# pingpongshow/RIA

Measured on AMD Instinct MI355X. Metric: frames/s demod+LDPC-decoded, OFDM QAM16 R1/2 1024-FFT, higher is better.
Workload: dtype f32; 1 GPU; OFDM QAM16 R1/2 + LDPC min-sum, Watterson moderate fading 20 dB, 4400000 frames (100000 per step per GPU), full decodeFixedFrame; frame_samples=18432, batch_per_gpu=100000, channel=2

## Files before the change

ria_amd/csrc/ldpc_fast.hip.h:

```cpp
#pragma once
#include <hip/hip_runtime.h>
#include <stdint.h>

#include <type_traits>

#include "../../include/ria_gpu.h"
#include "devmath.h"
#include "ldpc_kernels.hip.h"

namespace ria {

struct ShapeR12 {
    static constexpr int NR = 6, NC = 6;
    static constexpr int kCascadeWaves = 3;
    static constexpr int kCv = 24;
    static constexpr bool kStateExit = true;
    static constexpr int ne(int r) { constexpr int t[NR] = {6, 6, 5, 4, 2, 1}; return t[r]; }
    static constexpr int nm(int r) { constexpr int t[NR] = {6, 5, 4, 2, 1, 1}; return t[r]; }
    static constexpr int dv(int r) { constexpr int t[NC] = {5, 4, 4, 4, 4, 4}; return t[r]; }
};
struct ShapeR13 {
    static constexpr int NR = 6, NC = 6;
    static constexpr int kCascadeWaves = 3;
    static constexpr int kCv = 24;
// ... 43 lines not shown

template <class S>
struct ShapeInfo {
    static constexpr int row_off(int r) { int t = 0; for (int i = 0; i < r; ++i) t += S::ne(i); return t; }
    static constexpr int col_off(int r) { int t = 0; for (int i = 0; i < r; ++i) t += S::dv(i); return t; }
    static constexpr int mix_off(int r) { int t = 0; for (int i = 0; i < r; ++i) t += S::ne(i) - S::nm(i); return t; }
    static constexpr int TS = row_off(S::NR);
    static constexpr int TD = col_off(S::NC);
    static constexpr int TM = mix_off(S::NR);
    static constexpr int tot_word = 64 * TS;
    static constexpr int zero_word = tot_word + 64 * S::NC;
    static constexpr int dump_word = zero_word + 64;
    static constexpr int big_word = dump_word + 64;
    static constexpr int words = big_word + 64;
    static constexpr int lds_bytes = ((words < 1296 ? 1296 : words) * 4 + 15) & ~15;
    static constexpr int copy_words = 2 * S::NR + (S::NR + 1) / 2;
    static constexpr int exit_lds_bytes = lds_bytes + (S::kStateExit ? 256 * copy_words : 0);
};

template <int B, int E, class F>
__device__ __forceinline__ void static_for(F&& f) {
    if constexpr (B < E) {
        f(std::integral_constant<int, B>{});
        static_for<B + 1, E>(f);
    }
}

struct FastCode {
    int k, m, max_iter, bytes_per_cw;
    const uint16_t* row_addr;
    const uint16_t* col_addr;
    const uint16_t* check_at;
// ... 104 lines not shown
            if constexpr (N >= 5) { mid = med3_abs(w[4], lo, mid); lo = min_abs(w[4], lo); }
        }
    }
}
__device__ __forceinline__ uint32_t bfi(uint32_t mask, uint32_t a, uint32_t b) { return (mask & a) | (~mask & b); }

__device__ __forceinline__ float llr_canon(float x) {
    x = (x < 1e30f) ? x : 1e30f;
    x = (-1e30f < x) ? x : -1e30f;
    return x + 0.0f;
}

#ifndef RIA_SINGLE_PREFETCH
#define RIA_SINGLE_PREFETCH 2
#endif
constexpr int kExitFirst = 22, kExitStride = 24;
template <class S, int NCV = (kCvRegs ? 1024 : S::kCv), int PF = RIA_SINGLE_PREFETCH, bool EX = false>
__device__ inline int fast_decode(FastState<S>& st, const FastCode& c, unsigned char* __restrict__ lds,
                                  float factor, int max_iter, int lane, bool* ok, unsigned int* exits = nullptr) {
    using I = ShapeInfo<S>;
    static_assert(!EX || S::kStateExit, "the shape has no room for the state copy");
    const uint32_t lane4 = lds_addr(lds) + static_cast<uint32_t>(lane) * 4u;
    const uint32_t kAbs = 0x7fffffffu;
    const uint32_t m0base = lds_addr(lds);
    static_for<0, S::NR>([&](auto R_) __attribute__((always_inline)) {
        constexpr int r = decltype(R_)::value;
#pragma unroll
        for (int s = 0; s < S::ne(r); ++s) {
            const float v0 = 0.0f;
            if (I::row_off(r) + s < NCV) st.cv[I::row_off(r) + s] = v0;
            else lds_sf(lane4 + 256u * (I::row_off(r) + s), v0);
        }
    });
#pragma unroll
    for (int r = 0; r < S::NC; ++r) lds_sf(lane4 + 4u * (I::tot_word + 64 * r), st.li[r]);
    lds_sf(lane4 + 4u * I::zero_word, 0.0f);
    lds_sf(lane4 + 4u * I::big_word, kPadTotal);
#pragma unroll
    for (int r = 0; r < S::NR; ++r) { st.pv[r] = st.lp[r]; st.pt[r] = 0.0f; }
    wave_sync();
    float hi = __builtin_inff();
    int it = 0;
    bool success = false;
    auto iteration = [&](auto SNAP_) __attribute__((always_inline)) -> int {
        constexpr bool SNAP = decltype(SNAP_)::value;
        uint32_t syn = 0;
        uint32_t sb = 0, sd = 0;
        float tt[I::TS];
        auto gather_round = [&](auto G_) __attribute__((always_inline)) {
            constexpr int g = decltype(G_)::value;
            if constexpr (g < S::NR) {
#pragma unroll
                for (int s = 0; s < S::ne(g); ++s) tt[I::row_off(g) + s] = lds_f(st.rv[I::row_off(g) + s]);
            }
        };
        static_for<0, PF>([&](auto G_) __attribute__((always_inline)) { gather_round(G_); });
        static_for<0, S::NR>([&](auto R_) __attribute__((always_inline)) {
            constexpr int r = decltype(R_)::value;
            constexpr int NE = S::ne(r);
            constexpr int off = I::row_off(r);
            gather_round(std::integral_constant<int, r + PF>{});
            float t[NE], cold[NE];
// ... 27 lines not shown
            syn |= par;
            const uint32_t dS = bfi(kAbs, f2u(min1) ^ f2u(min2), sgn);
            float o[NE];
#pragma unroll
            for (int s = 0; s < NE; ++s) o[s] = u2f(dS ^ f2u(__builtin_amdgcn_fmed3f(v[s], min2, -min2))) * factor;
            lds_store_tid_n<NE, 256 * off, 256>(m0base, o);
            static_for<0, NE>([&](auto S_) __attribute__((always_inline)) {
                constexpr int s = decltype(S_)::value;
                if constexpr (off + s < NCV) st.cv[off + s] = o[s];
            });
            {
                const float c2v = u2f(dS ^ f2u(__builtin_amdgcn_fmed3f(pvr, min2, -min2))) * factor;
                const float tot = st.lp[r] + c2v;
                st.pv[r] = tot - c2v;
                st.pt[r] = tot;
                if constexpr (SNAP) {
                    static_assert(NE + 1 <= 8, "16 bits per round");
                    const uint32_t ma = f2u(min1 * factor) & kAbs, mb = f2u(min2 * factor) & kAbs;
                    uint32_t bits = (f2u(c2v) >> 31) | (((f2u(c2v) & kAbs) != ma) ? 2u : 0u);
#pragma unroll
                    for (int s = 0; s < NE; ++s) bits = (bits << 2) | (f2u(o[s]) >> 31) | (((f2u(o[s]) & kAbs) != ma) ? 2u : 0u);
                    const uint32_t ca = lane4 + static_cast<uint32_t>(I::lds_bytes) + 256u * (2 * r);
                    sd |= (f2u(lds_f(ca)) ^ ma) | (f2u(lds_f(ca + 256u)) ^ mb);
                    lds_sf(ca, u2f(ma));
                    lds_sf(ca + 256u, u2f(mb));
                    sb = (r & 1) ? (sb | (bits << 16)) : bits;
                    if constexpr ((r & 1) || r == S::NR - 1) {
                        const uint32_t cb = lane4 + static_cast<uint32_t>(I::lds_bytes) + 256u * (2 * S::NR + r / 2);
                        sd |= f2u(lds_f(cb)) ^ sb;
                        lds_sf(cb, u2f(sb));
                    }
                }
            }
        });
        if (it > 0 && __ballot(static_cast<int>(syn) < 0) == 0ull) return 1;
        if constexpr (SNAP) {
            if (it != kExitFirst && __ballot(sd != 0u) == 0ull) return 2;
        }
        hi = 50.0f;
        wave_sync();
        constexpr int NCE = []() constexpr { int n = 0; for (int r = 0; r < S::NC; ++r) if (S::dv(r) > 0) n = r + 1; return n; }();
        float totv[NCE > 0 ? NCE : 1];
        static_for<0, NCE>([&](auto R_) __attribute__((always_inline)) {
            constexpr int r = decltype(R_)::value;
            constexpr int DV = S::dv(r);
            constexpr int off = I::col_off(r);
            float cv[DV > 0 ? DV : 1];
#pragma unroll
            for (int d = 0; d < DV; ++d) cv[d] = lds_f(st.cs[off + d]);
            float tot = st.li[r];
#pragma unroll
            for (int d = 0; d < DV; ++d) tot = tot + cv[d];
            totv[r] = tot;
        });
        static_for<0, (NCE + 5) / 6>([&](auto G_) __attribute__((always_inline)) {
            constexpr int g0 = 6 * decltype(G_)::value, gn = (NCE - g0 < 6) ? NCE - g0 : 6;
            float tv[gn];
#pragma unroll
            for (int i = 0; i < gn; ++i) tv[i] = totv[g0 + i];
            lds_store_tid_n<gn, 4 * (I::tot_word + 64 * g0), 256>(m0base, tv);
        });
        wave_sync();
        return 0;
    };
    int snap_at = (EX && exits != nullptr) ? kExitFirst : 0x7fffffff;
    int status = 0;
    for (;;) {
        const int stop = snap_at < max_iter ? snap_at : max_iter;
        for (; it < stop; ++it) {
            status = iteration(std::false_type{});
            if (status != 0) break;
        }
        if (status != 0 || it >= max_iter) break;
        if constexpr (!EX) break;
        else {
            status = iteration(std::true_type{});
            if (status != 0) break;
            ++it;
            snap_at += kExitStride;
        }
    }
    if (status == 1) { success = true; --it; }
    if constexpr (EX) {
        if (status == 2) {
            if (lane == 0) atomicAdd(exits, 1u);
            *ok = false;
            return max_iter;
        }
    }
    if (!success) {
        uint32_t syn = 0;
        static_for<0, S::NR>([&](auto R_) __attribute__((always_inline)) {
            constexpr int r = decltype(R_)::value;
            constexpr int off = I::row_off(r);
            uint32_t par = f2u(st.pt[r]);
// ... 60 lines not shown
    uint8_t* info_out;
    ria_decode_status* status;
    const uint16_t* crc_bit;
    const uint16_t* crc_init;
    DecodeCtl* ctl;
    unsigned int* entries;
    unsigned int* best;
    unsigned int* list1;
    CwResult* res;
    uint8_t* res_bytes;
    CascadeWin* win;
    float* staged;
    unsigned int* l1idx;
    unsigned int* l1hash;
    uint32_t* seed_ws;
    int state_exit;
    __device__ unsigned int* exit_counter(int which) const { return state_exit ? &ctl->exits[which] : nullptr; }
};

constexpr int kStageFloats = 12 * 64;
constexpr int kStageFrameFloats = 2688;

constexpr float kIdleRowLlr = 1e30f;

template <class S>
__device__ inline void fast_gather_llr(FastState<S>& st, const FastCode& c, const float* fl, const uint16_t* gather,
                                       int cw, int lane) {
    lane = opaque_lane(lane);
#pragma unroll
    for (int r = 0; r < S::NC; ++r) {
        const uint32_t j = c.col_at[lane + 64 * r];
        st.li[r] = (j != 0xFFFFu) ? llr_canon(fl[gather[cw * 648 + j]]) : 0.0f;
// ... 12 lines not shown
#pragma unroll
    for (int r = 0; r < S::NC; ++r) st.li[r] = src[r * 64 + lane];
#pragma unroll
    for (int r = 0; r < S::NR; ++r) st.lp[r] = src[(S::NC + r) * 64 + lane];
}

__device__ inline void fast_publish(CwResult* res, unsigned fc, int f, bool ok, int it, int lane) {
    if (lane == 0) {
        res[fc].iters[f] = static_cast<uint16_t>(it);
        __hip_atomic_store(&res[fc].state[f], static_cast<uint8_t>(ok ? 2 : 1), __ATOMIC_RELAXED, __HIP_MEMORY_SCOPE_AGENT);
    }
}

template <class S, int NCV = S::kCv, bool EX = false>
__device__ inline void fast_unit(FastState<S>& st, const FastDecodeArgs& A, unsigned char* lds, unsigned fc, int f, int lane,
                                 const float* staged = nullptr, unsigned int* exits = nullptr) {
    const FastCode& c = A.c;
    if (staged) fast_load_staged(st, staged, lane);
    else fast_gather_llr(st, c, A.llr + static_cast<size_t>(fc >> 2) * A.llr_stride, A.gather, fc & 3, lane);
    bool ok;
    int it = fast_decode<S, NCV, RIA_SINGLE_PREFETCH, EX>(st, c, lds, kFactors[f], c.max_iter, lane, &ok, exits);
    if (ok) fast_pack(st, c, lds, A.res_bytes + (static_cast<size_t>(fc) * kNumFactors + f) * c.bytes_per_cw,
                      c.bytes_per_cw, lane);
    fast_publish(A.res, fc, f, ok, it, lane);
}

#ifndef RIA_PRIMARY_NCV
#define RIA_PRIMARY_NCV 0
#endif
template <class S>
__global__ __launch_bounds__(64) void fast_primary_kernel(FastDecodeArgs A) {
    extern __shared__ __attribute__((aligned(16))) unsigned char smem[];
    const int lane = threadIdx.x;
    const unsigned b = blockIdx.x, g = b >> 5, r = b & 31u, cw = r >> 3, x = r & 7u;
    const unsigned frame = 8u * g + x;
    if (frame >= static_cast<unsigned>(A.n_frames)) return;
// ... 55 lines not shown
                const uint32_t k = c.check_at[lane + 64 * (r - S::NC)];
                v = (k != 0xFFFFu) ? llr_canon(fr[A.gather[cw * 648 + c.k + k]]) : kIdleRowLlr;
            }
            dst[r * 64 + lane] = v;
        }
        if (wave == 0) {
            const uint32_t h = fast_hash16(fr, A.gather, cw, lane);
            if (lane == 0) A.l1hash[i] = h;
        }
    }
}

#ifndef RIA_EAGER_FACTORS
#define RIA_EAGER_FACTORS 0
#endif
template <class S, bool EX = false>
__global__ __launch_bounds__(64) void fast_phase0_kernel(FastDecodeArgs A) {
    extern __shared__ __attribute__((aligned(16))) unsigned char smem[];
    const int lane = threadIdx.x;
    const unsigned n_list1 = A.ctl->n_list1, total = n_list1 * 4u;
    if (blockIdx.x >= total) return;
    FastState<S> st;
    fast_load_tables(st, A.c, smem, lane);
    unsigned guard = 0;
    for (;;) {
        RIA_QUEUE_GUARD(guard, total, A.ctl)
        unsigned u = atomicAdd(&A.ctl->next_z, lane == 0 ? 1u : 0u);
        u = __builtin_amdgcn_readfirstlane(u);
        if (u >= total) break;
#if RIA_EAGER_FACTORS
        const unsigned entry = u >> 2;
        const int t = 1 + static_cast<int>(u & 3u);
        const unsigned fc = A.list1[entry];
#else
        const unsigned tq = u / n_list1, entry = u - tq * n_list1;
        const int t = 1 + static_cast<int>(tq);
        const unsigned fc = A.list1[entry];
        bool done = false;
        for (int k = 1; k < t; ++k) {
            const unsigned sk = __hip_atomic_load(&A.res[fc].state[k], __ATOMIC_RELAXED, __HIP_MEMORY_SCOPE_AGENT);
            done = done || __builtin_amdgcn_readfirstlane(sk) == 2u;
        }
        if (done) continue;
#endif
        fast_unit<S, S::kCv, EX>(st, A, smem, fc, t, lane, A.staged + static_cast<size_t>(entry) * kStageFloats,
                                 A.exit_counter(kExitsPhase0));
    }
}

__global__ void fast_chain_kernel(FastDecodeArgs A) {
    int frame = blockIdx.x * blockDim.x + threadIdx.x;
    if (frame >= A.n_frames) return;
    const int bpc = A.c.bytes_per_cw;
    int f = 0;
    ria_decode_status* s = A.status + frame;
    for (int cw = 0; cw < 4; ++cw) {
        const unsigned fc = static_cast<unsigned>(frame) * 4u + cw;
        const CwResult r = A.res[fc];
        int accept = -1, attempts = 1, iters = r.iters[f];
        if (r.state[f] == 2) accept = f;
        else {
// ... 52 lines not shown
    for (int r = 0; r < S::NC; ++r) {
        const uint32_t q = c.col_at[lane + 64 * r];
        const float nz = (noise && q != 0xFFFFu) ? normal[q] : 0.0f;
        st.li[r] = (q != 0xFFFFu) ? llr_canon(tf(base_i[r], nz)) : 0.0f;
    }
#pragma unroll
    for (int r = 0; r < S::NR; ++r) {
        const uint32_t i = c.check_at[lane + 64 * r];
        const float nz = (noise && i != 0xFFFFu) ? normal[c.k + i] : 0.0f;
        st.lp[r] = (i != 0xFFFFu) ? llr_canon(tf(base_p[r], nz)) : kIdleRowLlr;
    }
    wave_sync();
    return factor;
}

template <class S, bool EX = false>
__global__ __launch_bounds__(64) __attribute__((amdgpu_waves_per_eu(S::kCascadeWaves))) void fast_cascade_kernel(FastDecodeArgs A) {
    extern __shared__ __attribute__((aligned(16))) unsigned char smem[];
    const FastCode& c = A.c;
    const int lane = threadIdx.x;
    float* msg = reinterpret_cast<float*>(smem);
    const unsigned int n_entries = A.ctl->n_entries;
    const unsigned int total = n_entries * kCascadeGroups;
    if (total == 0) return;
    FastState<S> st;
    fast_load_tables(st, c, smem, lane);
    unsigned guard = 0;
    for (;;) {
        RIA_QUEUE_GUARD(guard, total, A.ctl)
        unsigned int u = atomicAdd(&A.ctl->next_unit, lane == 0 ? 1u : 0u);
        u = __builtin_amdgcn_readfirstlane(u);
// ... 10 lines not shown
            const unsigned int a = a0 + static_cast<unsigned>(j);
            if (a >= kRetryAttempts) break;
            if (j > 0) {
                b = __hip_atomic_load(&A.best[e], __ATOMIC_RELAXED, __HIP_MEMORY_SCOPE_AGENT);
                b = __builtin_amdgcn_readfirstlane(b);
                if (b < a) break;
            }
            fast_load_staged(st, A.staged + static_cast<size_t>(li) * kStageFloats, lane);
            float bi[S::NC], bp[S::NR];
#pragma unroll
            for (int r = 0; r < S::NC; ++r) bi[r] = st.li[r];
#pragma unroll
            for (int r = 0; r < S::NR; ++r) bp[r] = st.lp[r];
            float factor = fast_perturb(st, c, bi, bp, reinterpret_cast<uint32_t*>(msg), msg + 640, ws, j, static_cast<int>(a), lane);
            bool ok;
            const int it = fast_decode<S, (kCvRegs ? 1024 : S::kCv), RIA_SINGLE_PREFETCH, EX>(st, c, smem, factor, c.max_iter, lane, &ok,
                                                                                     A.exit_counter(kExitsCascade));
            if (!ok) continue;
            unsigned int prev = atomicMin(&A.best[e], lane == 0 ? a : 0xFFFFFFFFu);
            prev = __builtin_amdgcn_readfirstlane(prev);
            if (a < prev) {
                CascadeWin* w = A.win + e;
                bool mine = false;
                for (unsigned spin = 0; spin < (1u << 20); ++spin) {
                    unsigned got = atomicCAS(&w->lock, 0u, lane == 0 ? 1u : 0u);
                    got = __builtin_amdgcn_readfirstlane(got);
                    if (got == 0u) { mine = true; break; }
                    __builtin_amdgcn_s_sleep(1);
                }
                if (!mine) { if (lane == 0) atomicExch(&A.ctl->queue_fault, 1u); break; }
                __threadfence();
                unsigned int cur = __hip_atomic_load(&A.best[e], __ATOMIC_RELAXED, __HIP_MEMORY_SCOPE_AGENT);
// ... 154 lines not shown
```

ria_amd/csrc/recovery_kernels.hip.h:

```cpp
#pragma once
#include <hip/hip_runtime.h>
#include <stdint.h>

#include "fallback_relevance.hpp"
#include "ldpc_fast.hip.h"
#include "sort_exact.hpp"

namespace ria {

struct RecCtx {
    uint8_t* cw;
    uint8_t* fd;
    uint8_t* trial;
    Suspect* sus;
    int* stack;
    uint16_t* sd;
    uint16_t* lists;
    int sus_cap;
    unsigned long long* dbg;
    int bpc;
    const uint16_t* crc_bit;
    const uint16_t* crc_init;
    int lane;
};
// ... 414 lines not shown
    uint8_t* redec_bytes;
};

__global__ void recovery_list_kernel(RecoveryArgs R) {
    int frame = blockIdx.x * blockDim.x + threadIdx.x;
    if (frame >= R.d.n_frames || !R.d.status[frame].needs_recovery) return;
    R.flagged[atomicAdd(R.n_flagged, 1u)] = static_cast<unsigned>(frame);
    if (!R.list_units_now) return;
    for (int cw = 0; cw < 4; ++cw) {
        unsigned fc = static_cast<unsigned>(frame) * 4u + cw, mask = 0;
        for (int f = 1; f <= 4; ++f)
            if (R.d.res[fc].state[f] == 0) mask |= 1u << (f - 1);
        if (mask) R.list2[atomicAdd(R.n_list2, 1u)] = (fc << 4) | mask;
    }
}
template <class S, bool EX = false>
__global__ __launch_bounds__(64) void recovery_fill_kernel(RecoveryArgs R) {
    extern __shared__ __attribute__((aligned(16))) unsigned char smem[];
    const unsigned total = *R.n_list2 * 4u;
    if (blockIdx.x >= total) return;
    FastState<S> st;
    fast_load_tables(st, R.d.c, smem, threadIdx.x);
    unsigned guard = 0;
    for (;;) {
        RIA_QUEUE_GUARD(guard, total, R.d.ctl)
        unsigned u = atomicAdd(R.next_fill, threadIdx.x == 0 ? 1u : 0u);
        u = __builtin_amdgcn_readfirstlane(u);
        if (u >= total) break;
        const unsigned e = R.list2[u >> 2], fc = e >> 4;
        const int f = 1 + static_cast<int>(u & 3u);
        if (!((e >> (f - 1)) & 1u)) continue;
        const FastCode& c = R.d.c;
        const int lane = threadIdx.x;
        unsigned li = kNotListed;
        if (R.d.flags & (RIA_DECODE_PHASE0 | RIA_DECODE_PERTURB)) li = static_cast<unsigned>(__builtin_amdgcn_readfirstlane(static_cast<int>(R.d.l1idx[fc])));
        if (li != kNotListed) fast_load_staged(st, R.d.staged + static_cast<size_t>(li) * kStageFloats, lane);
        else fast_gather_llr(st, c, R.d.llr + static_cast<size_t>(fc >> 2) * R.d.llr_stride, R.d.gather, fc & 3, lane);
        bool ok;
        const int it = fast_decode<S, (kCvRegs ? 1024 : S::kCv), RIA_SINGLE_PREFETCH, EX>(st, c, smem, kFactors[f], c.max_iter, lane, &ok,
                                                                                 R.d.exit_counter(kExitsFill));
        if (ok) fast_pack(st, c, smem, R.d.res_bytes + (static_cast<size_t>(fc) * kNumFactors + f) * c.bytes_per_cw, c.bytes_per_cw, lane);
        fast_publish(R.d.res, fc, f, ok, it, lane);
    }
}
__global__ __launch_bounds__(256) void recovery_gather_kernel(RecoveryArgs R) {
    const unsigned q = blockIdx.x;
    if (q >= *R.n_flagged) return;
    const unsigned frame = R.flagged[q];
    const int bpc = R.d.c.bytes_per_cw, ib = 4 * bpc;
    for (int i = threadIdx.x; i < ib; i += 256) R.info_c[static_cast<size_t>(q) * ib + i] = R.d.info_out[static_cast<size_t>(frame) * ib + i];
    const float* fl = R.d.llr + static_cast<size_t>(frame) * R.d.llr_stride;
    for (int i = threadIdx.x; i < 4 * 648; i += 256) R.rows_c[static_cast<size_t>(q) * 4 * 648 + i] = fl[R.d.gather[i]];
    const int forder[4] = {2, 3, 4, 1};
    if (threadIdx.x < 16) {
        int at = threadIdx.x >> 2, cw = threadIdx.x & 3;
// ... 120 lines not shown
```

ria_amd/csrc/ria_gpu.hip:

```cpp
#include <hip/hip_runtime.h>

#include <cstdarg>
#include <cstdio>
#include <cstdlib>
#include <algorithm>
#include <cstring>
#include <map>
#include <memory>
#include <mutex>
#include <atomic>
#include <chrono>
#include <string>
#include <thread>
#include <vector>

#include "../../include/ria_gpu.h"
#include "host_tables.hpp"
#include "../host/link_adaptation.hpp"
#include "frame_recovery.hpp"
#include "ws_carve.hpp"
#include "device_buffers.hpp"
#include "ldpc_kernels.hip.h"
#include "ldpc_fast.hip.h"
#ifdef RIA_WITH_DUAL_DECODER
// ... 44 lines not shown
    DevBuf d_tx_const;
    DevBuf d_llr_ws;
    FastCode fast{};
    CoreTables ftab;
    DevBuf d_f[5];
    int wave_lds = 0;
    hipStream_t aux_stream[4] = {nullptr, nullptr, nullptr, nullptr};
    hipEvent_t aux_event[5] = {nullptr, nullptr, nullptr, nullptr, nullptr};
    DevBuf d_ctl;
    DevBuf d_seed_ws;
    DevBuf d_decode_ws;
    int ws_frames = 0;
    int split_parts = 0;
    int dual_decoder = 0;
    int fallback_queue_all = 0;
    int state_exit = 0;
    DevBuf d_hstage; PinBuf p_hstage; hipStream_t hstream = nullptr;
    int zc_lds_opted = 0, mc_lds_opted = 0, lts_lds_opted = 0;
    DevBuf d_rec_ws, d_rec_stage; PinBuf p_rec_stage;
    int rec_frames = 0, rec_host_frames = 0;
    Crc16Tables crc;
    DevBuf d_acq_ws; int acq_windows = 0; PinBuf p_acq_ctl;
    DevBuf d_macq_ws; PinBuf p_macq_ctl;
    DevBuf d_burst_ws; PinBuf p_burst_ctl;
    FastCode fast14{}; DevBuf d_f14[5]; int wave_lds14 = 0; bool have14 = false;
    DevBuf d_cw_perm[2];
    DevBuf d_df_ws; PinBuf p_df_ctl;
    std::vector<std::unique_ptr<ria_chase_pool_s>> chase_pools;
    DevBuf d_harq_ws, d_mdf_ws; PinBuf p_mdf_ctl;
};

// ... 66 lines not shown
};
static DecodeWs decode_ws_carve(Carver& c, size_t n_frames, size_t bytes_per_cw) {
    const size_t n4 = 4 * n_frames;
    DecodeWs w;
    w.entries = c.take<unsigned int>(n4);
    w.best = c.take<unsigned int>(n4);
    w.list1 = c.take<unsigned int>(n4);
    w.res = c.take<CwResult>(n4);
    w.res_bytes = c.take<uint8_t>(n4 * kNumFactors * bytes_per_cw);
    w.win = c.take<CascadeWin>(n4);
    w.staged = c.take<float>(n4 * kStageFloats);
    w.l1idx = c.take<unsigned int>(n4);
    w.l1hash = c.take<unsigned int>(n4);
    return w;
}
static hipError_t ensure_decode_ws(ria_gpu_handle h, int n_frames) {
    if (n_frames <= h->ws_frames && h->d_ctl && h->d_seed_ws) return hipSuccess;
    h->ws_frames = 0;
    hipError_t e;
    if (!h->d_ctl) {
        if ((e = h->d_ctl.reserve(kMaxParts * sizeof(DecodeCtl))) != hipSuccess) return e;
        if ((e = hipMemset(h->d_ctl.as<>(), 0, kMaxParts * sizeof(DecodeCtl))) != hipSuccess) { h->d_ctl.release(); return e; }
    }
    if ((e = h->d_seed_ws.reserve(static_cast<size_t>(kMaxParts) * persist_grid_size(false) * kSeedWsWords * sizeof(uint32_t))) != hipSuccess) return e;
    const size_t bpc = h->geo.bytes_per_codeword;
    if ((e = h->d_decode_ws.reserve(carved_size([&](Carver& c) { return decode_ws_carve(c, n_frames, bpc); }))) != hipSuccess) return e;
    h->ws_frames = n_frames;
    return hipSuccess;
}
template <class S, class F>
static void with_state_exit(ria_gpu_handle h, F&& f) {
    if constexpr (S::kStateExit) {
        if (h->state_exit) { f(std::true_type{}, ShapeInfo<S>::exit_lds_bytes); return; }
    }
    f(std::false_type{}, ShapeInfo<S>::lds_bytes);
}
static void set_fast_attributes(int rate, int wb) {
    dispatch_shape(rate, [&](auto s) {
        using S = decltype(s);
        (void)hipFuncSetAttribute(reinterpret_cast<const void*>(fast_primary_kernel<S>), hipFuncAttributeMaxDynamicSharedMemorySize, wb);
        (void)hipFuncSetAttribute(reinterpret_cast<const void*>(fast_phase0_kernel<S>), hipFuncAttributeMaxDynamicSharedMemorySize, wb);
        (void)hipFuncSetAttribute(reinterpret_cast<const void*>(fast_cascade_kernel<S>), hipFuncAttributeMaxDynamicSharedMemorySize, wb);
        if constexpr (S::kStateExit) {
            const int wbx = ShapeInfo<S>::exit_lds_bytes;
            (void)hipFuncSetAttribute(reinterpret_cast<const void*>(fast_phase0_kernel<S, true>), hipFuncAttributeMaxDynamicSharedMemorySize, wbx);
            (void)hipFuncSetAttribute(reinterpret_cast<const void*>(fast_cascade_kernel<S, true>), hipFuncAttributeMaxDynamicSharedMemorySize, wbx);
            (void)hipFuncSetAttribute(reinterpret_cast<const void*>(recovery_fill_kernel<S, true>), hipFuncAttributeMaxDynamicSharedMemorySize, wbx);
        }
        (void)hipFuncSetAttribute(reinterpret_cast<const void*>(fast_rows_kernel<S>), hipFuncAttributeMaxDynamicSharedMemorySize, wb);
        (void)hipFuncSetAttribute(reinterpret_cast<const void*>(fast_robust_kernel<S>), hipFuncAttributeMaxDynamicSharedMemorySize, wb);
#ifdef RIA_WITH_DUAL_DECODER
        (void)hipFuncSetAttribute(reinterpret_cast<const void*>(dual_phase0_kernel<S>), hipFuncAttributeMaxDynamicSharedMemorySize, DualInfo<S>::lds_bytes);
        (void)hipFuncSetAttribute(reinterpret_cast<const void*>(dual_cascade_kernel<S>), hipFuncAttributeMaxDynamicSharedMemorySize, DualInfo<S>::lds_bytes);
#endif
        (void)hipFuncSetAttribute(reinterpret_cast<const void*>(recovery_fill_kernel<S>), hipFuncAttributeMaxDynamicSharedMemorySize, wb);
    });
}

template <class F>
static void parallel_for(int n, F&& f) {
    int nt = static_cast<int>(std::min<unsigned>(16u, std::max(1u, std::thread::hardware_concurrency())));
    if (n < 64 || nt == 1) { for (int i = 0; i < n; ++i) f(i); return; }
    std::atomic<int> next{0};
// ... 82 lines not shown
    unsigned int* rctl = W.rctl + 8 * slot;
    R.n_flagged = rctl; R.n_list2 = rctl + 1; R.n_stage2 = rctl + 2; R.next_fill = rctl + 3; R.n_overflow = rctl + 4;
    R.n_queued = rctl + 5; R.queue_all = h->fallback_queue_all;
    R.flagged = W.flagged + ws_off; R.list2 = W.list2 + static_cast<size_t>(ws_off) * 16; R.stage2 = W.stage2 + ws_off;
    R.overflow = W.overflow + ws_off;
#ifdef RIA_DEBUG_STAMPS
    if (const char* e = getenv("RIA_DEBUG_REC_STAMPS")) R.dbg = reinterpret_cast<unsigned long long*>(strtoull(e, nullptr, 0));
#endif
    R.list_units_now = 0;
    if (hipMemsetAsync(rctl, 0, 32, s) != hipSuccess) return fail(h, RIA_ERR_HIP, "hipMemsetAsync failed");
    const int rl = recovery_lds_bytes(h->geo.bytes_per_codeword);
    hipLaunchKernelGGL(recovery_list_kernel, dim3((n_frames + 255) / 256), dim3(256), 0, s, R);
    hipLaunchKernelGGL(recovery_stage1_kernel, dim3(n_frames), dim3(64), rl, s, R);
    dispatch_shape(h->cfg.code_rate, [&](auto sh) {
        using S = decltype(sh);
        with_state_exit<S>(h, [&](auto ex, int lds) {
            hipLaunchKernelGGL((recovery_fill_kernel<S, decltype(ex)::value>), dim3(std::min(n_frames * 16, 3072)), dim3(64), lds, s, R);
        });
    });
    hipLaunchKernelGGL(recovery_stage2_kernel, dim3(n_frames), dim3(64), rl, s, R);
    hipLaunchKernelGGL(decode_fault_kernel, dim3((n_frames + 3) / 4), dim3(256), 0, s, static_cast<const DecodeCtl*>(D.ctl), D.status, D.info_out,
                       h->geo.bytes_per_codeword, n_frames);
    if (hipGetLastError() != hipSuccess) return fail(h, RIA_ERR_HIP, "recovery kernel launch failed");
    return RIA_OK;
}

static int run_crc_recovery_host(ria_gpu_handle h, const FastDecodeArgs& D, hipStream_t s) {
    static const bool tdbg = getenv("RIA_DEBUG_RECOVERY") != nullptr;
    auto now = []() { return std::chrono::duration<double, std::milli>(std::chrono::steady_clock::now().time_since_epoch()).count(); };
    const int n_frames = D.n_frames;
    double tA = now();
    hipError_t e0 = ensure_recovery_ws(h, std::max(n_frames, h->cfg.max_batch), true);
    if (e0 != hipSuccess) return fail(h, RIA_ERR_HIP, "recovery workspace: %s", hipGetErrorString(e0));
    const int bpc = h->geo.bytes_per_codeword, ib = h->geo.info_bytes_per_frame;
    RecoveryArgs R{};
    R.d = D;
    const RecoveryWs W = recovery_ws(h);
    const RecoveryStage Dv = recovery_stage(h, false), P = recovery_stage(h, true);
    R.n_flagged = W.rctl; R.n_list2 = W.rctl + 1; R.next_fill = W.rctl + 3;
    R.flagged = W.flagged; R.list2 = W.list2; R.list_units_now = 1;
    R.info_c = Dv.info_c; R.rows_c = Dv.rows_c; R.redec_ok = Dv.redec_ok; R.redec_bytes = Dv.redec_bytes;
#define R_TRY(expr) do { hipError_t e_ = (expr); if (e_ != hipSuccess) return fail(h, RIA_ERR_HIP, "%s: %s", #expr, hipGetErrorString(e_)); } while (0)
    R_TRY(hipMemsetAsync(W.rctl, 0, 16, s));
    hipLaunchKernelGGL(recovery_list_kernel, dim3((n_frames + 255) / 256), dim3(256), 0, s, R);
    const int wb = h->wave_lds;
    dispatch_shape(h->cfg.code_rate, [&](auto sh) {
        using S = decltype(sh);
        hipLaunchKernelGGL(recovery_fill_kernel<S>, dim3(std::min(n_frames * 16, 3072)), dim3(64), wb, s, R);
    });
    hipLaunchKernelGGL(recovery_gather_kernel, dim3(n_frames), dim3(256), 0, s, R);
    hipLaunchKernelGGL(recovery_status_gather_kernel, dim3((n_frames + 255) / 256), dim3(256), 0, s, W.rctl, W.flagged,
                       D.status, Dv.st_c);
    R_TRY(hipGetLastError());
    R_TRY(hipMemcpyAsync(P.rctl, W.rctl, 16, hipMemcpyDeviceToHost, s));
    R_TRY(hipStreamSynchronize(s));
    double tB = now();
    const int nf = static_cast<int>(P.rctl[0]);
    if (nf == 0) return RIA_OK;
    R_TRY(hipMemcpyAsync(P.flagged, W.flagged, static_cast<size_t>(nf) * 4, hipMemcpyDeviceToHost, s));
    R_TRY(hipMemcpyAsync(P.info_c, Dv.info_c, static_cast<size_t>(nf) * ib, hipMemcpyDeviceToHost, s));
    R_TRY(hipMemcpyAsync(P.rows_c, Dv.rows_c, static_cast<size_t>(nf) * 4 * 648 * 4, hipMemcpyDeviceToHost, s));
    R_TRY(hipMemcpyAsync(P.redec_ok, Dv.redec_ok, static_cast<size_t>(nf) * 16, hipMemcpyDeviceToHost, s));
    R_TRY(hipMemcpyAsync(P.redec_bytes, Dv.redec_bytes, static_cast<size_t>(nf) * 16 * bpc, hipMemcpyDeviceToHost, s));
// ... 274 lines not shown
    A.status = status_dev;
    A.crc_bit = h->d_crc_bit.as<const uint16_t>();
    A.crc_init = h->d_crc_init.as<const uint16_t>();
    A.ctl = h->d_ctl.as<DecodeCtl>() + slot;
    A.entries = W.entries + o4;
    A.best = W.best + o4;
    A.list1 = W.list1 + o4;
    A.res = W.res + o4;
    A.res_bytes = W.res_bytes + o4 * kNumFactors * bpc;
    A.win = W.win + o4;
    A.staged = W.staged + o4 * kStageFloats;
    A.l1idx = W.l1idx + o4;
    A.l1hash = W.l1hash + o4;
    A.seed_ws = h->d_seed_ws.as<uint32_t>() + static_cast<size_t>(slot) * persist_grid_size(false) * kSeedWsWords;
    dispatch_shape(h->cfg.code_rate, [&](auto sh) { A.state_exit = decltype(sh)::kStateExit ? h->state_exit : 0; });
    if ((e = hipMemsetAsync(A.ctl, 0, sizeof(DecodeCtl), s)) != hipSuccess)
        return fail(h, RIA_ERR_HIP, "hipMemsetAsync: %s", hipGetErrorString(e));
    const int wb = h->wave_lds;
#ifdef RIA_WITH_DUAL_DECODER
    static const bool dual_env = getenv("RIA_DUAL") && getenv("RIA_DUAL")[0] == '1';
    const bool dual = h->dual_decoder > 0 || (h->dual_decoder == 0 && dual_env);
#else
    const bool dual = false;
#endif
    const int persist_grid = persist_grid_size(dual);
    static const bool dbg = getenv("RIA_DEBUG_SYNC") != nullptr;
    auto stage = [&](const char* name) {
        if (!dbg) return;
        hipError_t e2 = hipStreamSynchronize(s);
        fprintf(stderr, "[ria_gpu] %s: %s\n", name, hipGetErrorString(e2));
// ... 2 lines not shown
    dispatch_shape(h->cfg.code_rate, [&](auto sh) {
        using S = decltype(sh);
        hipLaunchKernelGGL(fast_primary_kernel<S>, dim3(32 * ((n_frames + 7) / 8)), dim3(64), wb, s, A);
        stage("primary");
        hipLaunchKernelGGL(fast_mark_kernel, dim3((n_frames + 255) / 256), dim3(256), 0, s, A);
        stage("mark");
        if (flags & (RIA_DECODE_PHASE0 | RIA_DECODE_PERTURB)) {
            hipLaunchKernelGGL(fast_stage_kernel<S>, dim3(std::min(4 * n_frames, 8192)), dim3(256), 0, s, A);
            stage("stage");
        }
        if (flags & (RIA_DECODE_PHASE0 | RIA_DECODE_PERTURB)) {
#ifdef RIA_WITH_DUAL_DECODER
            if (dual) hipLaunchKernelGGL(dual_phase0_kernel<S>, dim3(std::min(n_frames * 8, persist_grid)), dim3(64), DualInfo<S>::lds_bytes, s, A);
            else
#endif
            with_state_exit<S>(h, [&](auto ex, int lds) {
                hipLaunchKernelGGL((fast_phase0_kernel<S, decltype(ex)::value>), dim3(std::min(n_frames * 16, persist_grid)), dim3(64), lds, s, A);
            });
        }
        stage("phase0");
        hipLaunchKernelGGL(fast_chain_kernel, dim3((n_frames + 255) / 256), dim3(256), 0, s, A);
        stage("chain");
        if (flags & RIA_DECODE_PERTURB) {
#ifdef RIA_WITH_DUAL_DECODER
            if (dual) hipLaunchKernelGGL(dual_cascade_kernel<S>, dim3(persist_grid), dim3(64), DualInfo<S>::lds_bytes, s, A);
            else
#endif
            with_state_exit<S>(h, [&](auto ex, int lds) {
                hipLaunchKernelGGL((fast_cascade_kernel<S, decltype(ex)::value>), dim3(persist_grid), dim3(64), lds, s, A);
            });
            stage("cascade");
            hipLaunchKernelGGL(fast_finalize_kernel, dim3(std::min((4 * n_frames + 255) / 256, 1024)), dim3(256), 0, s, A);
            stage("finalize");
        }
    });
    hipLaunchKernelGGL(frame_validate_kernel, dim3((n_frames + 3) / 4), dim3(256), 0, s, info_out_dev,
                       h->geo.bytes_per_codeword, n_frames, A.crc_bit, A.crc_init, status_dev, static_cast<const DecodeCtl*>(A.ctl));
    stage("validate");
    if (hipGetLastError() != hipSuccess) return fail(h, RIA_ERR_HIP, "decode kernel launch failed");
    if (flags & RIA_DECODE_CRC_RECOVER) return run_crc_recovery(h, A, s, slot, ws_off);
    return RIA_OK;
}

int ria_gpu_decode_batch(ria_gpu_handle h, const float* llr_dev, int llr_stride, int n_frames, uint32_t flags,
                         uint8_t* info_out_dev, ria_decode_status* status_dev, void* stream) {
// ... 1714 lines not shown
```

Measured before the change: 1.617 million frames/s.

## Enable repeated-state early exit by default using global-memory state snapshots

Replaces the LDS-based compressed snapshot exit with a full register-state snapshot (c2v messages plus per-row totals) written to a per-workgroup global workspace every stride of iterations, compared via an XOR checksum in LDS first and then a chunked inline-asm load/compare. The state exit is now on by default and compiled into the phase0, cascade and recovery-fill kernels, so decodes stuck in a fixed point stop early instead of running to max_iter. The extra LDS for the copy is no longer needed, so kernels use the base LDS size. In exchange it adds global stores and loads at snapshot points, an extra workspace allocation, and register pressure from holding the whole state in registers.

```diff
diff --git a/ria_amd/csrc/ldpc_fast.hip.h b/ria_amd/csrc/ldpc_fast.hip.h
--- a/ria_amd/csrc/ldpc_fast.hip.h
+++ b/ria_amd/csrc/ldpc_fast.hip.h
@@ -81,8 +81,7 @@
     static constexpr int big_word = dump_word + 64;
     static constexpr int words = big_word + 64;
     static constexpr int lds_bytes = ((words < 1296 ? 1296 : words) * 4 + 15) & ~15;
-    static constexpr int copy_words = 2 * S::NR + (S::NR + 1) / 2;
-    static constexpr int exit_lds_bytes = lds_bytes + (S::kStateExit ? 256 * copy_words : 0);
+    static constexpr int state_words = TS + 2 * S::NR;
 };
 
 template <int B, int E, class F>
@@ -217,12 +216,52 @@
 #ifndef RIA_SINGLE_PREFETCH
 #define RIA_SINGLE_PREFETCH 2
 #endif
+constexpr int kStateChunk = 12;
+constexpr int kStateWsWords = 36 * 64;
+#ifndef RIA_EXIT_FLIGHT
+#define RIA_EXIT_FLIGHT 3
+#endif
+template <int C, int N>
+__device__ __forceinline__ void state_store_chunk(const uint32_t* area, uint32_t lane4, const uint32_t (&w)[N]) {
+    static_assert(kStateChunk == 12 && 12 * C + 12 <= N && 256 * 11 < 4096, "twelve immediate offsets");
+    const uint32_t* base = area + 64 * kStateChunk * C;
+    asm volatile("global_store_dword %0, %1, %13\n\tglobal_store_dword %0, %2, %13 offset:256\n\t"
+                 "global_store_dword %0, %3, %13 offset:512\n\tglobal_store_dword %0, %4, %13 offset:768\n\t"
+                 "global_store_dword %0, %5, %13 offset:1024\n\tglobal_store_dword %0, %6, %13 offset:1280\n\t"
+                 "global_store_dword %0, %7, %13 offset:1536\n\tglobal_store_dword %0, %8, %13 offset:1792\n\t"
+                 "global_store_dword %0, %9, %13 offset:2048\n\tglobal_store_dword %0, %10, %13 offset:2304\n\t"
+                 "global_store_dword %0, %11, %13 offset:2560\n\tglobal_store_dword %0, %12, %13 offset:2816"
+                 : : "v"(lane4), "v"(w[12 * C]), "v"(w[12 * C + 1]), "v"(w[12 * C + 2]), "v"(w[12 * C + 3]), "v"(w[12 * C + 4]),
+                     "v"(w[12 * C + 5]), "v"(w[12 * C + 6]), "v"(w[12 * C + 7]), "v"(w[12 * C + 8]), "v"(w[12 * C + 9]),
+                     "v"(w[12 * C + 10]), "v"(w[12 * C + 11]), "s"(base) : "memory");
+}
+template <int C>
+__device__ __forceinline__ void state_load_chunk(const uint32_t* area, uint32_t lane4, uint32_t (&t)[kStateChunk]) {
+    const uint32_t* base = area + 64 * kStateChunk * C;
+    asm volatile("global_load_dword %0, %12, %13\n\tglobal_load_dword %1, %12, %13 offset:256\n\t"
+                 "global_load_dword %2, %12, %13 offset:512\n\tglobal_load_dword %3, %12, %13 offset:768\n\t"
+                 "global_load_dword %4, %12, %13 offset:1024\n\tglobal_load_dword %5, %12, %13 offset:1280\n\t"
+                 "global_load_dword %6, %12, %13 offset:1536\n\tglobal_load_dword %7, %12, %13 offset:1792\n\t"
+                 "global_load_dword %8, %12, %13 offset:2048\n\tglobal_load_dword %9, %12, %13 offset:2304\n\t"
+                 "global_load_dword %10, %12, %13 offset:2560\n\tglobal_load_dword %11, %12, %13 offset:2816"
+                 : "=&v"(t[0]), "=&v"(t[1]), "=&v"(t[2]), "=&v"(t[3]), "=&v"(t[4]), "=&v"(t[5]), "=&v"(t[6]), "=&v"(t[7]),
+                   "=&v"(t[8]), "=&v"(t[9]), "=&v"(t[10]), "=&v"(t[11])
+                 : "v"(lane4), "s"(base) : "memory");
+}
+__device__ __forceinline__ void state_wait_chunk(uint32_t (&t)[kStateChunk]) {
+    asm volatile("s_waitcnt vmcnt(0)"
+                 : "+v"(t[0]), "+v"(t[1]), "+v"(t[2]), "+v"(t[3]), "+v"(t[4]), "+v"(t[5]), "+v"(t[6]), "+v"(t[7]),
+                   "+v"(t[8]), "+v"(t[9]), "+v"(t[10]), "+v"(t[11]) : : "memory");
+}
 constexpr int kExitFirst = 22, kExitStride = 24;
 template <class S, int NCV = (kCvRegs ? 1024 : S::kCv), int PF = RIA_SINGLE_PREFETCH, bool EX = false>
 __device__ inline int fast_decode(FastState<S>& st, const FastCode& c, unsigned char* __restrict__ lds,
-                                  float factor, int max_iter, int lane, bool* ok, unsigned int* exits = nullptr) {
+                                  float factor, int max_iter, int lane, bool* ok, unsigned int* exits = nullptr,
+                                  uint32_t* state_ws = nullptr) {
     using I = ShapeInfo<S>;
-    static_assert(!EX || S::kStateExit, "the shape has no room for the state copy");
+    static_assert(!EX || S::kStateExit, "the shape has no repeated-state exit");
+    static_assert(!EX || (NCV >= I::TS && I::state_words % kStateChunk == 0 && I::state_words * 64 <= kStateWsWords),
+                  "the exit compares registers: every own c2v word must be in st.cv, in whole chunks, inside the workgroup's area");
     const uint32_t lane4 = lds_addr(lds) + static_cast<uint32_t>(lane) * 4u;
     const uint32_t kAbs = 0x7fffffffu;
     const uint32_t m0base = lds_addr(lds);
@@ -245,10 +284,8 @@
     float hi = __builtin_inff();
     int it = 0;
     bool success = false;
-    auto iteration = [&](auto SNAP_) __attribute__((always_inline)) -> int {
-        constexpr bool SNAP = decltype(SNAP_)::value;
+    auto iteration = [&]() __attribute__((always_inline)) -> int {
         uint32_t syn = 0;
-        uint32_t sb = 0, sd = 0;
         float tt[I::TS];
         auto gather_round = [&](auto G_) __attribute__((always_inline)) {
             constexpr int g = decltype(G_)::value;
@@ -306,29 +343,9 @@
                 const float tot = st.lp[r] + c2v;
                 st.pv[r] = tot - c2v;
                 st.pt[r] = tot;
-                if constexpr (SNAP) {
-                    static_assert(NE + 1 <= 8, "16 bits per round");
-                    const uint32_t ma = f2u(min1 * factor) & kAbs, mb = f2u(min2 * factor) & kAbs;
-                    uint32_t bits = (f2u(c2v) >> 31) | (((f2u(c2v) & kAbs) != ma) ? 2u : 0u);
-#pragma unroll
-                    for (int s = 0; s < NE; ++s) bits = (bits << 2) | (f2u(o[s]) >> 31) | (((f2u(o[s]) & kAbs) != ma) ? 2u : 0u);
-                    const uint32_t ca = lane4 + static_cast<uint32_t>(I::lds_bytes) + 256u * (2 * r);
-                    sd |= (f2u(lds_f(ca)) ^ ma) | (f2u(lds_f(ca + 256u)) ^ mb);
-                    lds_sf(ca, u2f(ma));
-                    lds_sf(ca + 256u, u2f(mb));
-                    sb = (r & 1) ? (sb | (bits << 16)) : bits;
-                    if constexpr ((r & 1) || r == S::NR - 1) {
-                        const uint32_t cb = lane4 + static_cast<uint32_t>(I::lds_bytes) + 256u * (2 * S::NR + r / 2);
-                        sd |= f2u(lds_f(cb)) ^ sb;
-                        lds_sf(cb, u2f(sb));
-                    }
-                }
             }
         });
         if (it > 0 && __ballot(static_cast<int>(syn) < 0) == 0ull) return 1;
-        if constexpr (SNAP) {
-            if (it != kExitFirst && __ballot(sd != 0u) == 0ull) return 2;
-        }
         hi = 50.0f;
         wave_sync();
         constexpr int NCE = []() constexpr { int n = 0; for (int r = 0; r < S::NC; ++r) if (S::dv(r) > 0) n = r + 1; return n; }();
@@ -352,25 +369,58 @@
             for (int i = 0; i < gn; ++i) tv[i] = totv[g0 + i];
             lds_store_tid_n<gn, 4 * (I::tot_word + 64 * g0), 256>(m0base, tv);
         });
+        if constexpr (EX) {
+#pragma unroll
+            for (int r = 0; r < S::NR; ++r) asm volatile("" : "+v"(st.pv[r]), "+v"(st.pt[r]));
+        }
         wave_sync();
         return 0;
     };
     int snap_at = (EX && exits != nullptr) ? kExitFirst : 0x7fffffff;
     int status = 0;
     for (;;) {
-        const int stop = snap_at < max_iter ? snap_at : max_iter;
+        const int stop = snap_at < max_iter ? snap_at + 1 : max_iter;
         for (; it < stop; ++it) {
-            status = iteration(std::false_type{});
+            status = iteration();
             if (status != 0) break;
         }
-        if (status != 0 || it >= max_iter) break;
+        if (status != 0 || it <= snap_at) break;
         if constexpr (!EX) break;
         else {
-            status = iteration(std::true_type{});
-            if (status != 0) break;
-            ++it;
+            uint32_t w[I::state_words];
+#pragma unroll
+            for (int i = 0; i < I::TS; ++i) w[i] = f2u(st.cv[i]);
+#pragma unroll
+            for (int r = 0; r < S::NR; ++r) { w[I::TS + r] = f2u(st.pv[r]); w[I::TS + S::NR + r] = f2u(st.pt[r]); }
+            const uint32_t g4 = static_cast<uint32_t>(lane) * 4u;
+            constexpr int NCH = I::state_words / kStateChunk;
+            uint32_t sum = 0;
+#pragma unroll
+            for (int i = 0; i < I::state_words; ++i) sum ^= w[i];
+            const uint32_t sum_at = lane4 + 4u * I::dump_word;
+            if (snap_at != kExitFirst && __ballot(f2u(lds_f(sum_at)) != sum) == 0ull) {
+                uint32_t sd = 0;
+                static_for<0, (NCH + RIA_EXIT_FLIGHT - 1) / RIA_EXIT_FLIGHT>([&](auto G_) __attribute__((always_inline)) {
+                    constexpr int c0 = RIA_EXIT_FLIGHT * decltype(G_)::value, cn = (NCH - c0 < RIA_EXIT_FLIGHT) ? NCH - c0 : RIA_EXIT_FLIGHT;
+                    uint32_t t[cn][kStateChunk];
+                    static_for<0, cn>([&](auto C_) __attribute__((always_inline)) { state_load_chunk<c0 + decltype(C_)::value>(state_ws, g4, t[decltype(C_)::value]); });
+                    static_for<0, cn>([&](auto C_) __attribute__((always_inline)) { state_wait_chunk(t[decltype(C_)::value]); });
+#pragma unroll
+                    for (int c = 0; c < cn; ++c)
+#pragma unroll
+                        for (int j = 0; j < kStateChunk; ++j) sd |= t[c][j] ^ w[kStateChunk * (c0 + c) + j];
+                });
+                if (__ballot(sd != 0u) == 0ull) { status = 2; break; }
+            }
+            if (snap_at + kExitStride < max_iter) {
+                static_for<0, NCH>([&](auto C_) __attribute__((always_inline)) { state_store_chunk<decltype(C_)::value>(state_ws, g4, w); });
+                lds_sf(sum_at, u2f(sum));
+            }
             snap_at += kExitStride;
         }
+    }
+    if constexpr (EX) {
+        if (exits != nullptr) asm volatile("s_waitcnt vmcnt(0)" ::: "memory");
     }
     if (status == 1) { success = true; --it; }
     if constexpr (EX) {
@@ -461,8 +511,10 @@
     unsigned int* l1idx;
     unsigned int* l1hash;
     uint32_t* seed_ws;
+    uint32_t* state_ws;
     int state_exit;
     __device__ unsigned int* exit_counter(int which) const { return state_exit ? &ctl->exits[which] : nullptr; }
+    __device__ uint32_t* state_area() const { return state_ws + static_cast<size_t>(blockIdx.x) * kStateWsWords; }
 };
 
 constexpr int kStageFloats = 12 * 64;
@@ -505,12 +557,12 @@
 
 template <class S, int NCV = S::kCv, bool EX = false>
 __device__ inline void fast_unit(FastState<S>& st, const FastDecodeArgs& A, unsigned char* lds, unsigned fc, int f, int lane,
-                                 const float* staged = nullptr, unsigned int* exits = nullptr) {
+                                 const float* staged = nullptr, unsigned int* exits = nullptr, uint32_t* state_ws = nullptr) {
     const FastCode& c = A.c;
     if (staged) fast_load_staged(st, staged, lane);
     else fast_gather_llr(st, c, A.llr + static_cast<size_t>(fc >> 2) * A.llr_stride, A.gather, fc & 3, lane);
     bool ok;
-    int it = fast_decode<S, NCV, RIA_SINGLE_PREFETCH, EX>(st, c, lds, kFactors[f], c.max_iter, lane, &ok, exits);
+    int it = fast_decode<S, NCV, RIA_SINGLE_PREFETCH, EX>(st, c, lds, kFactors[f], c.max_iter, lane, &ok, exits, state_ws);
     if (ok) fast_pack(st, c, lds, A.res_bytes + (static_cast<size_t>(fc) * kNumFactors + f) * c.bytes_per_cw,
                       c.bytes_per_cw, lane);
     fast_publish(A.res, fc, f, ok, it, lane);
@@ -596,7 +648,7 @@
 #ifndef RIA_EAGER_FACTORS
 #define RIA_EAGER_FACTORS 0
 #endif
-template <class S, bool EX = false>
+template <class S>
 __global__ __launch_bounds__(64) void fast_phase0_kernel(FastDecodeArgs A) {
     extern __shared__ __attribute__((aligned(16))) unsigned char smem[];
     const int lane = threadIdx.x;
@@ -625,8 +677,8 @@
         }
         if (done) continue;
 #endif
-        fast_unit<S, S::kCv, EX>(st, A, smem, fc, t, lane, A.staged + static_cast<size_t>(entry) * kStageFloats,
-                                 A.exit_counter(kExitsPhase0));
+        fast_unit<S, S::kCv, S::kStateExit>(st, A, smem, fc, t, lane, A.staged + static_cast<size_t>(entry) * kStageFloats,
+                                            A.exit_counter(kExitsPhase0), A.state_area());
     }
 }
 
@@ -709,7 +761,7 @@
     return factor;
 }
 
-template <class S, bool EX = false>
+template <class S>
 __global__ __launch_bounds__(64) __attribute__((amdgpu_waves_per_eu(S::kCascadeWaves))) void fast_cascade_kernel(FastDecodeArgs A) {
     extern __shared__ __attribute__((aligned(16))) unsigned char smem[];
     const FastCode& c = A.c;
@@ -750,8 +802,8 @@
             for (int r = 0; r < S::NR; ++r) bp[r] = st.lp[r];
             float factor = fast_perturb(st, c, bi, bp, reinterpret_cast<uint32_t*>(msg), msg + 640, ws, j, static_cast<int>(a), lane);
             bool ok;
-            const int it = fast_decode<S, (kCvRegs ? 1024 : S::kCv), RIA_SINGLE_PREFETCH, EX>(st, c, smem, factor, c.max_iter, lane, &ok,
-                                                                                     A.exit_counter(kExitsCascade));
+            const int it = fast_decode<S, (kCvRegs ? 1024 : S::kCv), RIA_SINGLE_PREFETCH, S::kStateExit>(st, c, smem, factor, c.max_iter, lane, &ok,
+                                                                                                A.exit_counter(kExitsCascade), A.state_area());
             if (!ok) continue;
             unsigned int prev = atomicMin(&A.best[e], lane == 0 ? a : 0xFFFFFFFFu);
             prev = __builtin_amdgcn_readfirstlane(prev);
diff --git a/ria_amd/csrc/recovery_kernels.hip.h b/ria_amd/csrc/recovery_kernels.hip.h
--- a/ria_amd/csrc/recovery_kernels.hip.h
+++ b/ria_amd/csrc/recovery_kernels.hip.h
@@ -452,7 +452,7 @@
         if (mask) R.list2[atomicAdd(R.n_list2, 1u)] = (fc << 4) | mask;
     }
 }
-template <class S, bool EX = false>
+template <class S>
 __global__ __launch_bounds__(64) void recovery_fill_kernel(RecoveryArgs R) {
     extern __shared__ __attribute__((aligned(16))) unsigned char smem[];
     const unsigned total = *R.n_list2 * 4u;
@@ -475,8 +475,8 @@
         if (li != kNotListed) fast_load_staged(st, R.d.staged + static_cast<size_t>(li) * kStageFloats, lane);
         else fast_gather_llr(st, c, R.d.llr + static_cast<size_t>(fc >> 2) * R.d.llr_stride, R.d.gather, fc & 3, lane);
         bool ok;
-        const int it = fast_decode<S, (kCvRegs ? 1024 : S::kCv), RIA_SINGLE_PREFETCH, EX>(st, c, smem, kFactors[f], c.max_iter, lane, &ok,
-                                                                                 R.d.exit_counter(kExitsFill));
+        const int it = fast_decode<S, (kCvRegs ? 1024 : S::kCv), RIA_SINGLE_PREFETCH, S::kStateExit>(st, c, smem, kFactors[f], c.max_iter, lane, &ok,
+                                                                                            R.d.exit_counter(kExitsFill), R.d.state_area());
         if (ok) fast_pack(st, c, smem, R.d.res_bytes + (static_cast<size_t>(fc) * kNumFactors + f) * c.bytes_per_cw, c.bytes_per_cw, lane);
         fast_publish(R.d.res, fc, f, ok, it, lane);
     }
diff --git a/ria_amd/csrc/ria_gpu.hip b/ria_amd/csrc/ria_gpu.hip
--- a/ria_amd/csrc/ria_gpu.hip
+++ b/ria_amd/csrc/ria_gpu.hip
@@ -82,7 +82,8 @@
     int split_parts = 0;
     int dual_decoder = 0;
     int fallback_queue_all = 0;
-    int state_exit = 0;
+    DevBuf d_state_ws;
+    int state_exit = 1;
     DevBuf d_hstage; PinBuf p_hstage; hipStream_t hstream = nullptr;
     int zc_lds_opted = 0, mc_lds_opted = 0, lts_lds_opted = 0;
     DevBuf d_rec_ws, d_rec_stage; PinBuf p_rec_stage;
@@ -179,8 +180,12 @@
     w.l1hash = c.take<unsigned int>(n4);
     return w;
 }
+constexpr int kFillGrid = 3072;
+static int state_grid_size() { return std::max(persist_grid_size(false), kFillGrid); }
 static hipError_t ensure_decode_ws(ria_gpu_handle h, int n_frames) {
-    if (n_frames <= h->ws_frames && h->d_ctl && h->d_seed_ws) return hipSuccess;
+    bool state_exit_rate = false;
+    dispatch_shape(h->cfg.code_rate, [&](auto sh) { state_exit_rate = decltype(sh)::kStateExit; });
+    if (n_frames <= h->ws_frames && h->d_ctl && h->d_seed_ws && (h->d_state_ws || !state_exit_rate)) return hipSuccess;
     h->ws_frames = 0;
     hipError_t e;
     if (!h->d_ctl) {
@@ -188,17 +193,12 @@
         if ((e = hipMemset(h->d_ctl.as<>(), 0, kMaxParts * sizeof(DecodeCtl))) != hipSuccess) { h->d_ctl.release(); return e; }
     }
     if ((e = h->d_seed_ws.reserve(static_cast<size_t>(kMaxParts) * persist_grid_size(false) * kSeedWsWords * sizeof(uint32_t))) != hipSuccess) return e;
+    if (state_exit_rate &&
+        (e = h->d_state_ws.reserve(static_cast<size_t>(kMaxParts) * state_grid_size() * kStateWsWords * sizeof(uint32_t))) != hipSuccess) return e;
     const size_t bpc = h->geo.bytes_per_codeword;
     if ((e = h->d_decode_ws.reserve(carved_size([&](Carver& c) { return decode_ws_carve(c, n_frames, bpc); }))) != hipSuccess) return e;
     h->ws_frames = n_frames;
     return hipSuccess;
-}
-template <class S, class F>
-static void with_state_exit(ria_gpu_handle h, F&& f) {
-    if constexpr (S::kStateExit) {
-        if (h->state_exit) { f(std::true_type{}, ShapeInfo<S>::exit_lds_bytes); return; }
-    }
-    f(std::false_type{}, ShapeInfo<S>::lds_bytes);
 }
 static void set_fast_attributes(int rate, int wb) {
     dispatch_shape(rate, [&](auto s) {
@@ -206,12 +206,6 @@
         (void)hipFuncSetAttribute(reinterpret_cast<const void*>(fast_primary_kernel<S>), hipFuncAttributeMaxDynamicSharedMemorySize, wb);
         (void)hipFuncSetAttribute(reinterpret_cast<const void*>(fast_phase0_kernel<S>), hipFuncAttributeMaxDynamicSharedMemorySize, wb);
         (void)hipFuncSetAttribute(reinterpret_cast<const void*>(fast_cascade_kernel<S>), hipFuncAttributeMaxDynamicSharedMemorySize, wb);
-        if constexpr (S::kStateExit) {
-            const int wbx = ShapeInfo<S>::exit_lds_bytes;
-            (void)hipFuncSetAttribute(reinterpret_cast<const void*>(fast_phase0_kernel<S, true>), hipFuncAttributeMaxDynamicSharedMemorySize, wbx);
-            (void)hipFuncSetAttribute(reinterpret_cast<const void*>(fast_cascade_kernel<S, true>), hipFuncAttributeMaxDynamicSharedMemorySize, wbx);
-            (void)hipFuncSetAttribute(reinterpret_cast<const void*>(recovery_fill_kernel<S, true>), hipFuncAttributeMaxDynamicSharedMemorySize, wbx);
-        }
         (void)hipFuncSetAttribute(reinterpret_cast<const void*>(fast_rows_kernel<S>), hipFuncAttributeMaxDynamicSharedMemorySize, wb);
         (void)hipFuncSetAttribute(reinterpret_cast<const void*>(fast_robust_kernel<S>), hipFuncAttributeMaxDynamicSharedMemorySize, wb);
 #ifdef RIA_WITH_DUAL_DECODER
@@ -324,9 +318,7 @@
     hipLaunchKernelGGL(recovery_stage1_kernel, dim3(n_frames), dim3(64), rl, s, R);
     dispatch_shape(h->cfg.code_rate, [&](auto sh) {
         using S = decltype(sh);
-        with_state_exit<S>(h, [&](auto ex, int lds) {
-            hipLaunchKernelGGL((recovery_fill_kernel<S, decltype(ex)::value>), dim3(std::min(n_frames * 16, 3072)), dim3(64), lds, s, R);
-        });
+        hipLaunchKernelGGL(recovery_fill_kernel<S>, dim3(std::min(n_frames * 16, kFillGrid)), dim3(64), h->wave_lds, s, R);
     });
     hipLaunchKernelGGL(recovery_stage2_kernel, dim3(n_frames), dim3(64), rl, s, R);
     hipLaunchKernelGGL(decode_fault_kernel, dim3((n_frames + 3) / 4), dim3(256), 0, s, static_cast<const DecodeCtl*>(D.ctl), D.status, D.info_out,
@@ -356,7 +348,7 @@
     const int wb = h->wave_lds;
     dispatch_shape(h->cfg.code_rate, [&](auto sh) {
         using S = decltype(sh);
-        hipLaunchKernelGGL(recovery_fill_kernel<S>, dim3(std::min(n_frames * 16, 3072)), dim3(64), wb, s, R);
+        hipLaunchKernelGGL(recovery_fill_kernel<S>, dim3(std::min(n_frames * 16, kFillGrid)), dim3(64), wb, s, R);
     });
     hipLaunchKernelGGL(recovery_gather_kernel, dim3(n_frames), dim3(256), 0, s, R);
     hipLaunchKernelGGL(recovery_status_gather_kernel, dim3((n_frames + 255) / 256), dim3(256), 0, s, W.rctl, W.flagged,
@@ -661,6 +653,7 @@
     A.l1hash = W.l1hash + o4;
     A.seed_ws = h->d_seed_ws.as<uint32_t>() + static_cast<size_t>(slot) * persist_grid_size(false) * kSeedWsWords;
     dispatch_shape(h->cfg.code_rate, [&](auto sh) { A.state_exit = decltype(sh)::kStateExit ? h->state_exit : 0; });
+    A.state_ws = h->d_state_ws ? h->d_state_ws.as<uint32_t>() + static_cast<size_t>(slot) * state_grid_size() * kStateWsWords : nullptr;
     if ((e = hipMemsetAsync(A.ctl, 0, sizeof(DecodeCtl), s)) != hipSuccess)
         return fail(h, RIA_ERR_HIP, "hipMemsetAsync: %s", hipGetErrorString(e));
     const int wb = h->wave_lds;
@@ -693,9 +686,7 @@
             if (dual) hipLaunchKernelGGL(dual_phase0_kernel<S>, dim3(std::min(n_frames * 8, persist_grid)), dim3(64), DualInfo<S>::lds_bytes, s, A);
             else
 #endif
-            with_state_exit<S>(h, [&](auto ex, int lds) {
-                hipLaunchKernelGGL((fast_phase0_kernel<S, decltype(ex)::value>), dim3(std::min(n_frames * 16, persist_grid)), dim3(64), lds, s, A);
-            });
+            hipLaunchKernelGGL(fast_phase0_kernel<S>, dim3(std::min(n_frames * 16, persist_grid)), dim3(64), wb, s, A);
         }
         stage("phase0");
         hipLaunchKernelGGL(fast_chain_kernel, dim3((n_frames + 255) / 256), dim3(256), 0, s, A);
@@ -705,9 +696,7 @@
             if (dual) hipLaunchKernelGGL(dual_cascade_kernel<S>, dim3(persist_grid), dim3(64), DualInfo<S>::lds_bytes, s, A);
             else
 #endif
-            with_state_exit<S>(h, [&](auto ex, int lds) {
-                hipLaunchKernelGGL((fast_cascade_kernel<S, decltype(ex)::value>), dim3(persist_grid), dim3(64), lds, s, A);
-            });
+            hipLaunchKernelGGL(fast_cascade_kernel<S>, dim3(persist_grid), dim3(64), wb, s, A);
             stage("cascade");
             hipLaunchKernelGGL(fast_finalize_kernel, dim3(std::min((4 * n_frames + 255) / 256, 1024)), dim3(256), 0, s, A);
             stage("finalize");
```

New measurement: 1.651 million frames/s, median of 6. +2.1%, better.
